# mims-harvard/GNNDelete

Hardware: AMD Instinct MI355X
Metric: Del-op train iters/sec (higher is better)
Workload: dtype f32; 1 GPU; synth-collab GCN 2-layer, 5.0% IN edge deletion, full-graph Del step (both_layerwise, mse_mean); num_nodes=235868, in_dim=128, hidden_dim=128, out_dim=64, train_edges_undirected=2122296, df_edges=53057, sdf_edges=1602188, spmm_nnz=1838056, S1=178921, S2=188697, hip_graph=True, matrix_products=fp32 matrix instruction (v_mfma_f32_32x32x2_f32), parallelism=single, ranks_seen=1

## Files before the change

gnndelete_amd/_lib.py:

```python
import ctypes
import os
import re

_HERE = os.path.dirname(os.path.abspath(__file__))
LIB_PATH = os.environ.get('GNNDELETE_HIP_LIB') or os.path.join(_HERE, 'lib', 'libgnndelete_hip.so')
HEADER_PATH = os.path.join(os.path.dirname(_HERE), 'include', 'gnndelete_hip.h')

_i32, _i64, _f32, _f64, _p = ctypes.c_int32, ctypes.c_int64, ctypes.c_float, ctypes.c_double, ctypes.c_void_p

ABI_VERSION = 9

PROTOTYPES = {
    'gd_abi_version': (ctypes.c_int, []),
    'gd_last_error_string': (ctypes.c_char_p, []),
    'gd_build_source_hash': (ctypes.c_char_p, []),
    'gd_matrix_split': (ctypes.c_int, []),
    'gd_set_matrix_split': (ctypes.c_int, [ctypes.c_int]),
    'gd_csr_from_coo_workspace': (_i64, [_i32, _i64]),
    'gd_csr_from_coo': (ctypes.c_int, [_p, _p, _i64, _i32, _p, _p, _p, _p, _p, _i64, _p]),
    'gd_gcn_norm_f32': (ctypes.c_int, [_p, _p, _i32, _p, _p]),
    'gd_spmm_csr_f32': (ctypes.c_int, [_p, _p, _p, _p, _i64, _p, _i64, _p, _f32, _i32, _i32, _p]),
    'gd_spmm_csr_balanced_f32': (ctypes.c_int, [_p, _i32, _p, _i32, _p, _p, _p, _i64, _p, _i64, _p, _f32, _p, _p, _i32,
                                                _i32, _i32, _p, _p]),
    'gd_spmm_csr_onepass_f32': (ctypes.c_int, [_p, _i32, _p, _p, _p, _i64, _p, _i64, _p, _f32, _p, _i32, _i32, _i32, _p, _p]),
# ... 47 lines not shown
    'gd_rowpair_mse_f32': (ctypes.c_int, [_p, _i64, _p, _i64, _i32, _p, _p, _i32, _p, _p, _p, _p, _i64, _i32,
                                          _p, _p, _p]),
    'gd_rowtarget_mse_workspace': (_i64, [_i32]),
    'gd_rowtarget_mse_f32': (ctypes.c_int, [_p, _i64, _p, _i32, _p, _p, _p, _p, _i32, _p, _i64, _p, _p, _p]),
    'gd_rowtarget_mse_pair_covers': (ctypes.c_int32, [_i32, _i32]),
    'gd_rowtarget_mse_pair_f32': (ctypes.c_int, [_p, _i64, _p, _i32, _p, _p, _p, _p, _i32, _p, _i64, _p, _p, _i64, _p, _i32, _p, _p, _p, _p, _i32, _p, _i64, _p, _p]),
    'gd_gemm_f32_workspace': (_i64, [_i32, _i32, _i32]),
    'gd_gemm_f32': (ctypes.c_int, [_p, _i64, _p, _i32, _p, _i32, _i32, _p, _p, _i64, _p, _p]),
    'gd_edge_dot_f32': (ctypes.c_int, [_p, _i64, _i32, _p, _p, _p, _i64, _p, _i64, _p, _p]),
    'gd_edge_dot_bwd_f32': (ctypes.c_int, [_p, _i64, _i32, _p, _p, _p, _i64, _p, _p, _i64, _p, _i64, _p]),
    'gd_rows_gemm_wgrad_adam_f32': (ctypes.c_int, [_p, _i64, _p, _p, _i64, _p, _p, _p, _i32, _i32, _i32, _p, _i32, _p,
                                                   _p, _p, _p, _p, _f64, _f64, _f64, _f64, _p]),
    'gd_rows_gemm_wgrad_blocks': (_i32, [_i32]),
    'gd_rows_gemm_wgrad_loss_f32': (ctypes.c_int, [_p, _i64, _p, _p, _i64, _p, _p, _p, _p, _p, _p, _i32, _i32, _i32, _p, _i32,
                                                   _p, _p, _p, _p, _p, _p, _f64, _f64, _f64, _f64, _p]),
    'gd_del_loss_bwd_blocks': (_i32, [_i32]),
    'gd_del_loss_bwd_f32': (ctypes.c_int, [_p, _i64, _p, _i32, _p, _i32, _p, _p, _p, _p, _p, _i64, _p, _i64, _p, _p]),
    'gd_del_loss_bwd_wgrad_f32': (ctypes.c_int, [_p, _i64, _p, _i32, _p, _i32, _p, _p, _p, _p, _p, _i64, _p, _i64, _p, _p, _p]),
    'gd_del_loss_bwd_wgrad_parts': (ctypes.c_int32, [_i32, _i32]),
    'gd_del_loss_bwd_wgrad_parts_f32': (ctypes.c_int, [_p, _i64, _p, _i32, _p, _i32, _p, _p, _p, _p, _p, _i64, _p, _i64, _p, _p, _i32, _p]),
    'gd_del1_loss_wgrad_covers': (ctypes.c_int32, [_i32, _i32]),
    'gd_del1_loss_wgrad_parts': (ctypes.c_int32, [_i32]),
    'gd_del1_chain_loss_wgrad_f32': (ctypes.c_int, [_p, _i64, _p, _i32, _p, _i32, _p, _i64, _p, _p, _p, _p, _p, _p, _i64, _i32, _p, _p, _p, _p, _p, _p, _p, _i32, _p]),
    'gd_del1_loss_wgrad_f32': (ctypes.c_int, [_p, _i64, _p, _i32, _p, _i32, _p, _i64, _p, _p, _p, _p, _p, _p, _i64, _p, _p, _i32, _p]),
    'gd_rowtarget_mse_blocks': (_i32, [_i32]),
    'gd_loss_finalize_f32': (ctypes.c_int, [_p, _i32, _p, _i32, _p, _p, _i32, _p, _p, _p]),
    'gd_pairs_sigmoid_mse_workspace': (_i64, [_i32, _i32]),
    'gd_pairs_sigmoid_mse_f32': (ctypes.c_int, [_p, _i64, _p, _i32, _i32, _p, _i64, _f32, _p, _p, _p, _p]),
    'gd_edgeprob_dec_workspace': (_i64, [_i64, _i32]),
    'gd_edgeprob_dec_f32': (ctypes.c_int, [_p, _i64, _i64, _i32, _p, _i64, _p, _i64, _i64, _f32, _p, _p, _p, _p, _p, _p, _p]),
    'gd_edge_incidence_workspace': (_i64, [_i64, _i64]),
    'gd_edge_incidence': (ctypes.c_int, [_p, _p, _i64, _i64, _p, _p, _p, _p, _i64, _p]),
    'gd_rows_add_f32': (ctypes.c_int, [_p, _i64, _i64, _p, _i32, _p, _i64, _f32, _i32, _p]),
    'gd_edgeprob_record_f32': (ctypes.c_int, [_p, _p, _f32, _f32, _p, _i32, _p, _p]),
    'gd_adam_at_f32': (ctypes.c_int, [_p, _p, _p, _p, _p, _i64, _f64, _f64, _f64, _f64, _p]),
    'gd_adam_f32': (ctypes.c_int, [_p, _p, _p, _p, _p, _i64, _f64, _f64, _f64, _f64, _p]),
    'gd_segment_softmax_f32': (ctypes.c_int, [_p, _p, _i32, _p, _p]),
    'gd_segment_softmax_bwd_f32': (ctypes.c_int, [_p, _p, _p, _i32, _p, _p]),
    'gd_rowpair_dot_f32': (ctypes.c_int, [_p, _i64, _p, _p, _i64, _p, _i64, _i32, _p, _p]),
    'gd_spmm_csr_onepass_aux_f32': (ctypes.c_int, [_p, _i32, _p, _p, _p, _p, _i64, _p, _i64, _p, _i32, _i32, _i32, _p, _p]),
    'gd_typed_wgrad_f32': (ctypes.c_int, [_p, _i32, _p, _p, _p, _p, _i64, _p, _i64, _i32, _i32, _i32, _p, _p]),
    'gd_typed_edge_dot_f32': (ctypes.c_int, [_p, _p, _p, _i64, _p, _i64, _p, _i64, _p, _i32, _i32, _i32, _p, _p]),
    'gd_comm_unique_id': (ctypes.c_int, [_p]),
    'gd_comm_init': (ctypes.c_int, [_p, _i32, _i32, ctypes.POINTER(ctypes.c_void_p)]),
    'gd_comm_destroy': (ctypes.c_int, [_p]),
    'gd_allreduce_f32': (ctypes.c_int, [_p, _i64, _p, _p]),
# ... 62 lines not shown
```

gnndelete_amd/csrc/common.h:

```cpp
#pragma once
#include <hip/hip_runtime.h>
#include <stdarg.h>
#include <stdint.h>
#include <stdio.h>

#include "gnndelete_hip.h"

namespace gd {

constexpr int kWave = 64;

char* error_buffer();
int matrix_split();
int ws_cu_count();
int rows_gemm_ws_try(const float* in, int64_t ld_in, const int32_t* idx, int32_t n_sel, const float* w, int32_t d_in, int32_t d_out,
                     int32_t trans_w, const float* bias, int32_t relu_in, const uint32_t* gate_bits, uint32_t* sign_out, float* out,
                     int64_t ld_out, float* save_in, void* stream, const float* in_alt, const uint8_t* sel, const float* u1,
                     const float* u2, float* o1, float* o2);

inline int fail(int code, const char* fmt, ...) {
  va_list ap;
  va_start(ap, fmt);
  vsnprintf(error_buffer(), 256, fmt, ap);
  va_end(ap);
// ... 32 lines not shown
  return __uint_as_float(r[0]) + __uint_as_float(r[1]);
}
__device__ __forceinline__ float xor16_sum(float v) {
  const auto r = __builtin_amdgcn_permlane16_swap(__float_as_uint(v), __float_as_uint(v), false, false);
  return __uint_as_float(r[0]) + __uint_as_float(r[1]);
}
template <int CTRL>
__device__ __forceinline__ float dpp_add(float v) {
  return v + __int_as_float(__builtin_amdgcn_update_dpp(0, __float_as_int(v), CTRL, 0xF, 0xF, true));
}
template <int LPR>
__device__ __forceinline__ float lanes_sum(float v) {
  if (LPR >= 2) v = dpp_add<0xB1>(v);
  if (LPR >= 4) v = dpp_add<0x4E>(v);
  if (LPR >= 8) v = dpp_add<0x141>(v);
  if (LPR >= 16) v = dpp_add<0x140>(v);
  if (LPR >= 32) v = xor16_sum(v);
  if (LPR >= 64) v = xor32_sum(v);
  return v;
}

template <int LPR>
__device__ __forceinline__ float4 f4_group_sum(float4 a) {
#pragma unroll
  for (int off = LPR; off < 8; off <<= 1) a = f4_add(a, f4_shfl_xor(a, off));
  if (LPR <= 8) a = make_float4(dpp_add<0x128>(a.x), dpp_add<0x128>(a.y), dpp_add<0x128>(a.z), dpp_add<0x128>(a.w));
  if (LPR <= 16) a = make_float4(xor16_sum(a.x), xor16_sum(a.y), xor16_sum(a.z), xor16_sum(a.w));
  if (LPR <= 32) a = make_float4(xor32_sum(a.x), xor32_sum(a.y), xor32_sum(a.z), xor32_sum(a.w));
  return a;
}
__device__ __forceinline__ float wave_sum(float v) {
#pragma unroll
  for (int off = 32; off > 0; off >>= 1) v += __shfl_xor(v, off);
  return v;
}

struct AdamScalars { float w1, b2, c2, neg_step, rs, eps; };
__device__ __forceinline__ AdamScalars adam_scalars(double lr, double beta1, double beta2, double eps, int t) {
  const double bc1 = 1.0 - pow(beta1, (double)t), bc2 = 1.0 - pow(beta2, (double)t);
  AdamScalars s;
  s.w1 = (float)(1.0 - beta1);
  s.b2 = (float)beta2;
  s.c2 = (float)(1.0 - beta2);
  s.neg_step = (float)(-(lr / bc1));
  s.rs = (float)sqrt(bc2);
  s.eps = (float)eps;
  return s;
}
__device__ __forceinline__ void adam_update(float& p, float& m, float& v, float g, const AdamScalars& s) {
#pragma clang fp contract(off)
  m = __builtin_fmaf(g - m, s.w1, m);
// ... 20 lines not shown
```

gnndelete_amd/csrc/del_fused.hip:

```cpp
#include <stdlib.h>

#include "common.h"

namespace gd {

using f32x16 = __attribute__((ext_vector_type(16))) float;

struct DelLoss {
  const int32_t* slot;
  const float* tm;
  const float* coef;
  const float* cnt_signed;
  float* partials;
};

template <int NT, bool WG>
__global__ __launch_bounds__(256, (NT == 2 && WG) ? 1 : 2) void del_loss_bwd_kernel(const float* __restrict__ p, int64_t ld_p,
                                                              const int32_t* __restrict__ idx, int32_t n_sel,
                                                              const float* __restrict__ w, DelLoss loss,
                                                              float* __restrict__ dz, int64_t ld_dz,
                                                              float* __restrict__ dp, int64_t ld_dp,
                                                              float* __restrict__ wg_partials) {
  constexpr int D = 32 * NT;
  constexpr int PB = D + 4;
// ... 532 lines not shown
  __syncthreads();
  for (int slot = blockIdx.x; slot < n_part; slot += gridDim.x) {
    float* const out = wg_partials + (int64_t)slot * D * D;
    const bool mine = slot == (int)blockIdx.x;
    for (int e = tid; e < D * D; e += 256) {
      const int i = e >> 7, c = e & 127, hf = c >> 6, ch = c & 63;
      out[e] = mine ? red[hf * D * H + i * H + ch] + red[(2 + hf) * D * H + i * H + ch] : 0.f;
    }
  }
  ls0 = wave_sum(ls0);
  ls1 = wave_sum(ls1);
  if (lane == 0) { lred[0][wave] = ls0; lred[1][wave] = ls1; }
  __syncthreads();
  if (tid == 0) {
    for (int slot = blockIdx.x; slot < n_part; slot += gridDim.x) {
      const bool mine = slot == (int)blockIdx.x;
      loss.partials[2 * slot + 0] = mine ? (lred[0][0] + lred[0][1]) + (lred[0][2] + lred[0][3]) : 0.f;
      loss.partials[2 * slot + 1] = mine ? (lred[1][0] + lred[1][1]) + (lred[1][2] + lred[1][3]) : 0.f;
    }
  }
}

struct ChainRank1 { const float* ra; const float* ua; const float* rb; const float* ub; };
template <bool RANK1>
__global__ __launch_bounds__(256) __attribute__((amdgpu_waves_per_eu(1, 1))) void del1_chain_ws_kernel(
    const float* __restrict__ p, int64_t ld_p, const int32_t* __restrict__ idx, int32_t n_sel, const float* __restrict__ w,
    float* __restrict__ z, int64_t ld_z, uint32_t* __restrict__ sign_io, DelLoss loss, const float* __restrict__ dt, int64_t ld_dt,
    const float* __restrict__ w_next, float* __restrict__ wg_partials, int32_t n_part, ChainRank1 r1) {
  constexpr int D = 128, H = 64, PTP = 144, PTZ = 80;
  constexpr int kTiles = 4 * (16 * PTP + 16 * PTZ);
  extern __shared__ __attribute__((aligned(16))) float wl[];
  __shared__ float lred[2][4];
  const int tid = threadIdx.x, lane = tid & 63;
  const int wave = __builtin_amdgcn_readfirstlane(tid >> 6);
  const int half = wave & 1, pair = wave >> 1, cb = H * half;
  const int r = lane & 15, kq = lane >> 4;
  float* const tp = wl + wave * (16 * PTP + 16 * PTZ);
  float* const tz = tp + 16 * PTP;
  float4* const wimg = reinterpret_cast<float4*>(wl + kTiles);
  float4* const w2img = wimg + 2 * 4 * 8 * 64;
  {
    float4 fv[16];
#pragma unroll
    for (int it = 0; it < 16; ++it) {
      const int e = tid + 256 * it;
      const int ln = e & 63, i_ = (e >> 6) & 7, t_ = (e >> 9) & 3, h_ = e >> 11;
      const float* src = w + (int64_t)(16 * i_ + 4 * (ln >> 4)) * D + 64 * h_ + 16 * t_ + (ln & 15);
// ... 33 lines not shown
  if (RANK1) {
#pragma unroll
    for (int t = 0; t < 4; ++t) {
      ua4[t] = *reinterpret_cast<const float4*>(r1.ua + cb + 16 * t + 4 * kq);
      ub4[t] = *reinterpret_cast<const float4*>(r1.ub + cb + 16 * t + 4 * kq);
    }
  }
  uint2 old_bits;
  float cf_raw, cn_raw;
  int32_t ls_cur;
  auto fetch_targets = [&](int32_t u) {
    const int uc = max(u, 0);
    const float* trow = loss.tm + (int64_t)uc * D + cb + 4 * kq;
#pragma unroll
    for (int t = 0; t < 4; ++t) tv[t] = *reinterpret_cast<const float4*>(trow + 16 * t);
    cf_raw = loss.coef[uc];
    cn_raw = loss.cnt_signed[uc];
    ls_cur = u;
  };
  auto fetch_rows = [&](int32_t row, int u) {
    const float4* src = reinterpret_cast<const float4*>(p + (int64_t)row * ld_p + 4 * kq);
#pragma unroll
    for (int i = 0; i < 8; ++i) x[i] = src[4 * i];
    const float4* dsrc = reinterpret_cast<const float4*>(dt + (int64_t)row * ld_dt + 4 * kq);
#pragma unroll
    for (int i = 0; i < 4; ++i) dv[i] = dsrc[4 * i];
    old_bits = *reinterpret_cast<const uint2*>(sign_io + (int64_t)slot_of(u) * 4 + 2 * half);
    if (RANK1) { ra_row = r1.ra[row]; rb_row = r1.rb[row]; }
  };
  if (u_lo < u_hi) {
    fetch_rows(row_n, u_lo);
    fetch_targets(ls_n);
    for (int u = u_lo; u < u_hi; ++u) {
      const int32_t row = row_n;
      const int s_a = min(u, n_units - 1) * 16 + r;
      const bool live = s_a < n_sel;
      const float livef = live ? 1.f : 0.f;
      row_n = row_nn;
      ls_n = ls_nn;
      row_nn = idx[slot_of(u + 2)];
      ls_nn = loss.slot[slot_of(u + 2)];
      f32x4w acc[4], dacc[4];
      {
        float4 wq[2][4];
#pragma unroll
        for (int t = 0; t < 4; ++t) wq[0][t] = wmine[(t * 8) * 64];
#pragma unroll
        for (int i = 0; i < 8; ++i) {
          if (i + 1 < 8) {
#pragma unroll
// ... 256 lines not shown
  GD_REQUIRE(aligned16(p) && aligned16(z) && aligned16(tm) && aligned16(w) && (!g_add || aligned16(g_add)) && aligned16(wgrad_partials),
             GD_E_ALIGN, "%s: unaligned", name);
  GD_REQUIRE(p != z && g_add != z, GD_E_DIM, "%s: z must not alias p or g_add (the two waves of a pair read whole rows)", name);
  hipStream_t s = (hipStream_t)stream;
  const DelLoss loss{loss_slot, tm, coef, cnt_signed, loss_partials};
  GD_REQUIRE(n_part >= 1 && n_part <= gd_rows_gemm_wgrad_blocks(n_sel), GD_E_DIM,
             "%s: n_part=%d outside [1, gd_rows_gemm_wgrad_blocks(n_sel)=%d]", name, n_part, gd_rows_gemm_wgrad_blocks(n_sel));
  const int grid = ws_cu_count() < n_part ? ws_cu_count() : n_part;
  constexpr int kLds = 4 * 128 * 64 * 4;
  if (g_add) {
    static const hipError_t a1 = hipFuncSetAttribute(reinterpret_cast<const void*>(&del1_loss_wgrad_ws_kernel<true>), hipFuncAttributeMaxDynamicSharedMemorySize, kLds);
    if (a1 != hipSuccess) return fail(-(int)a1, "%s: %s", name, hipGetErrorString(a1));
    hipLaunchKernelGGL((del1_loss_wgrad_ws_kernel<true>), dim3(grid), dim3(256), kLds, s, p, ld_p, idx, n_sel, w, z, ld_z, sign_out, loss, g_add,
                       ld_gadd, wgrad_partials, n_part);
  } else {
    static const hipError_t a0 = hipFuncSetAttribute(reinterpret_cast<const void*>(&del1_loss_wgrad_ws_kernel<false>), hipFuncAttributeMaxDynamicSharedMemorySize, kLds);
    if (a0 != hipSuccess) return fail(-(int)a0, "%s: %s", name, hipGetErrorString(a0));
    hipLaunchKernelGGL((del1_loss_wgrad_ws_kernel<false>), dim3(grid), dim3(256), kLds, s, p, ld_p, idx, n_sel, w, z, ld_z, sign_out, loss, nullptr,
                       0, wgrad_partials, n_part);
  }
  return launched("del1_loss_wgrad_ws");
}

extern "C" int gd_del1_chain_loss_wgrad_f32(const float* p, int64_t ld_p, const int32_t* idx, int32_t n_sel, const float* w, int32_t d,
                                            float* z, int64_t ld_z, uint32_t* sign_io, const int32_t* loss_slot, const float* tm,
                                            const float* coef, const float* cnt_signed, const float* dt, int64_t ld_dt, int32_t d_next,
                                            const float* w_next, const float* row_a, const float* col_a, const float* row_b,
                                            const float* col_b, float* loss_partials, float* wgrad_partials, int32_t n_part,
                                            void* stream) {
  using namespace gd;
  const char* name = "gd_del1_chain_loss_wgrad_f32";
  if (n_sel == 0) return GD_OK;
  GD_REQUIRE(p && idx && w && z && sign_io && loss_slot && tm && coef && cnt_signed && dt && w_next && loss_partials && wgrad_partials, GD_E_NULL,
             "%s: null pointer", name);
  GD_REQUIRE(d == 128 && d_next == 64, GD_E_DIM, "%s: widths %d / %d must be 128 / 64", name, d, d_next);
  GD_REQUIRE(ld_p >= d && ld_z >= d && ld_dt >= d_next && ld_p % 4 == 0 && ld_z % 4 == 0 && ld_dt % 4 == 0, GD_E_DIM, "%s: bad row strides", name);
  GD_REQUIRE(aligned16(p) && aligned16(z) && aligned16(tm) && aligned16(dt) && aligned16(wgrad_partials) && (reinterpret_cast<uintptr_t>(sign_io) & 7u) == 0,
             GD_E_ALIGN, "%s: unaligned", name);
  GD_REQUIRE(p != z && dt != z, GD_E_DIM, "%s: z must not alias p or dt", name);
  GD_REQUIRE(n_part >= 1 && n_part <= gd_rows_gemm_wgrad_blocks(n_sel), GD_E_DIM,
             "%s: n_part=%d outside [1, gd_rows_gemm_wgrad_blocks(n_sel)=%d]", name, n_part, gd_rows_gemm_wgrad_blocks(n_sel));
  const DelLoss loss{loss_slot, tm, coef, cnt_signed, loss_partials};
  const int grid = ws_cu_count() < n_part ? ws_cu_count() : n_part;
  constexpr int kLds = (4 * (16 * 144 + 16 * 80) + 128 * 128 + 64 * 128) * 4;
  const bool rank1 = row_a || col_a || row_b || col_b;
  GD_REQUIRE(!rank1 || (row_a && col_a && row_b && col_b && aligned16(col_a) && aligned16(col_b)), GD_E_NULL,
             "%s: the rank-1 terms come as four pointers (row_a, col_a, row_b, col_b; 16-byte aligned column vectors)", name);
  const ChainRank1 r1{row_a, col_a, row_b, col_b};
  if (rank1) {
    static const hipError_t at = hipFuncSetAttribute(reinterpret_cast<const void*>(&del1_chain_ws_kernel<true>), hipFuncAttributeMaxDynamicSharedMemorySize, kLds);
    if (at != hipSuccess) return fail(-(int)at, "%s: %s", name, hipGetErrorString(at));
    hipLaunchKernelGGL(del1_chain_ws_kernel<true>, dim3(grid), dim3(256), kLds, (hipStream_t)stream, p, ld_p, idx, n_sel, w, z, ld_z, sign_io, loss, dt,
                       ld_dt, w_next, wgrad_partials, n_part, r1);
  } else {
    static const hipError_t at = hipFuncSetAttribute(reinterpret_cast<const void*>(&del1_chain_ws_kernel<false>), hipFuncAttributeMaxDynamicSharedMemorySize, kLds);
    if (at != hipSuccess) return fail(-(int)at, "%s: %s", name, hipGetErrorString(at));
    hipLaunchKernelGGL(del1_chain_ws_kernel<false>, dim3(grid), dim3(256), kLds, (hipStream_t)stream, p, ld_p, idx, n_sel, w, z, ld_z, sign_io, loss, dt,
                       ld_dt, w_next, wgrad_partials, n_part, r1);
  }
  return launched("del1_chain_ws");
}
```

gnndelete_amd/engine.py:

```python
import os

import torch

from . import _lib, ops
from ._lib import check, ptr, stream_ptr
from .graph import graph_for
from .nn import GATConv, GCNConv, GINConv, RGCNConv, SAGEConv

LOSS_TYPES = ('both_all', 'both_layerwise', 'only2_layerwise', 'only2_all', 'only1')


def _loss_coefficients(loss_type, alpha):
    if loss_type in ('both_all', 'both_layerwise', 'only2_layerwise'):
        return alpha, 1.0 - alpha
    return alpha, 1.0


class _LayerTerms:

    def __init__(self, pos_edge, neg_edge, ni_mask, z_ori, coef_r, coef_l, reduction, row_range=None, d_norm=None):
        device = z_ori.device
        d = z_ori.shape[1]
        dn = d if d_norm is None else int(d_norm)
        pos, neg = pos_edge.to(device).long(), neg_edge.to(device).long()
# ... 316 lines not shown
        self._tail = (t1.folded and self.t2.folded and self.s1 > 0 and self.s2 > 0
                      and loss_type in ('both_layerwise', 'both_all') and not self._overlap and self.h % 2 == 0 and self.o % 2 == 0
                      and os.environ.get('GD_NO_STEP_TAIL') != '1'
                      and ((self._fuse_loss1 and self._fuse_l2)
                           or (self.h in (32, 64, 128) and self.o in (32, 64, 128) and os.environ.get('GD_TAIL_FUSED_ONLY') != '1')))
        self._tail_acc = [0, 0]
        self._arrive = torch.zeros(2, dtype=torch.int32, device=dev)
        self._fuse_wg2 = self._tail and self._fuse_l2 and os.environ.get('GD_NO_FUSED_WGRAD2') != '1'
        if self._fuse_wg2:
            self._lp2 = torch.zeros(2 * max(1, _lib.lib().gd_rows_gemm_wgrad_blocks(self.s2) + self.t2.outside_blocks()), **f32)
            self._lp2_blocks = _lib.lib().gd_del_loss_bwd_wgrad_parts(self.s2, self.o)
        self._fuse_del1 = bool(self._tail and self._fuse_loss1 and self._split1 and loss_type in ('both_layerwise', 'only1')
                               and _lib.lib().gd_del1_loss_wgrad_covers(self.s1, self.h))
        if self._fuse_del1:
            self._lp1_blocks = _lib.lib().gd_del1_loss_wgrad_parts(self.s1)
        self._chain1 = bool(self._fuse_del1 and loss_type == 'both_layerwise' and isinstance(conv2, (GCNConv, GINConv))
                            and self.h == 128 and self.o == 64 and os.environ.get('GD_DEL1_CHAIN') != '0')
        self._gat_bufs = None
        if (self._fuse_del1 and loss_type == 'both_layerwise' and isinstance(conv2, GATConv) and self.h == 128 and self.o == 64
                and self._mfma_weight(conv2.lin_src.weight) and os.environ.get('GD_NO_GAT_RANK1_EPILOGUE') != '1'
                and os.environ.get('GD_DEL1_CHAIN') != '0'):
            self._chain1 = True
            self._gat_bufs = {'dh': torch.zeros(n, self.o, **f32), 'da_src': torch.zeros(n, **f32), 'da_dst': torch.zeros(n, **f32)}
        self._dt2_keep = torch.zeros(n, self.o, **f32) if (self._chain1 and self._gat_bufs is None) else None
        self._side_w1 = bool(self._tail and self._fuse_loss1 and not self._fuse_del1 and loss_type == 'both_layerwise'
                             and self.s1 > 0 and not self._overlap and os.environ.get('GD_SMALL_SIDE_W1') == '1')
        if self._side_w1 and self._side is None:
            self._side = torch.cuda.Stream(device=dev)
        self._out_pair = bool(self._out1 and self._out2 and self._fuse_loss1 and self._fuse_l2 and loss_type != 'only2_all'
                              and _lib.lib().gd_rowtarget_mse_pair_covers(self.h, self.o) and os.environ.get('GD_NO_LOSS_PAIR') != '1')
        self._mode = {GCNConv: 'gcn', GINConv: 'gin', GATConv: 'gat', SAGEConv: 'sage', RGCNConv: 'rgcn'}[type(conv2)]
        self._gat_dots = os.environ.get('GD_NO_GAT_DOTS') != '1'
        self._gat_r1 = None
        if self._mode == 'gat':
            w2_ = conv2.lin_src.weight.detach()
            self._gat_r1 = ((conv2.att_src.detach().reshape(1, -1) @ w2_).reshape(-1).float().contiguous(),
                            (conv2.att_dst.detach().reshape(1, -1) @ w2_).reshape(-1).float().contiguous())
        if self._mode == 'rgcn':
            from .graph import TypedNodeCSR
            self.typed = TypedNodeCSR(edge_index, edge_type.to(dev), n, conv2.num_relations)
            self.typed_s1 = None
            if getattr(self, '_rgcn_rows_only', False) and self.s1 > 0:
                in1 = torch.zeros(n, dtype=torch.bool, device=dev)
                in1[self.idx1.long()] = True
                self.typed_s1 = self.typed.restrict_bwd(in1)
            self.graph = None
            self._hbuf = torch.zeros(n, self.h, **f32)
            self._dxbuf = torch.zeros(n, self.h, **f32)
            for c_, din, dout, tr in ((conv1, self.x.shape[1], self.h, 0), (conv2, self.h, self.o, 0), (conv2, self.o, self.h, 1)):
                if int(_lib.lib().gd_rgcn_tile_kl(din, dout, c_.num_blocks or 1, tr)) > 0 and os.environ.get('GD_RGCN_NODE_MAJOR') != '1':
                    tg_ = self.typed_s1 if (tr and self.typed_s1 is not None) else self.typed
                    if ops.rgcn_wave_form(din, dout, c_.num_blocks or 1, n, din) and self.typed.num_relations < 65536:
                        tg_.wave_plan(bool(tr))
                    else:
                        tg_.tile_plan(bool(tr))
                    ops.rgcn_packed_weight(c_.weight.detach(), c_.num_blocks or 1, din, dout, tr)
        else:
            gmode = {'gcn': 'gcn', 'gin': 'sum', 'gat': 'gat', 'sage': 'mean'}[self._mode]
            self.graph = graph_for(edge_index, n, gmode)
        if self._mode == 'sage':
            self._w2cat = torch.cat([conv2.lin_l.weight.detach(), conv2.lin_r.weight.detach()], 0).contiguous()
        self._rows_only = False
        gin_ok = self._mode == 'gin' and conv1.nn.out_features <= conv1.nn.in_features and conv2.nn.out_features <= conv2.nn.in_features
        if (affected_rows_only and (self._mode in ('gcn', 'gat', 'sage') or gin_ok) and self._split2 and self.s2 > 0
                and not self._out1 and not self._out2):
            g = self.graph
            in2 = torch.zeros(n, dtype=torch.bool, device=dev)
            in2[self.idx2.long()] = True
            in1_rows = torch.zeros(n, dtype=torch.bool, device=dev)
            in1_rows[self.idx1.long()] = True
            deg = (g.rowptr[1:] - g.rowptr[:-1]).long()
            erow = torch.repeat_interleave(torch.arange(n, device=dev), deg)
            closed = bool(in2[g.col.long()[in2[erow]]].all()) and bool(in2[self.idx1.long()].all())
            deg_t = (g.rowptr_t[1:] - g.rowptr_t[:-1]).long()
            erow_t = torch.repeat_interleave(torch.arange(n, device=dev), deg_t)
            closed = closed and bool(in2[g.col_t.long()[in1_rows[erow_t]]].all())
            if closed:
                from .graph import SplitPlan
                self._plan2 = SplitPlan(g.rowptr, rows=self.idx2)
                self._plan_t1 = SplitPlan(g.rowptr_t, rows=self.idx1)
                self._t1buf = torch.zeros(n, self.h, **f32)
                self._t1rbuf = torch.zeros(n, self.h, **f32) if self._mode == 'sage' else None
                self._t2buf = torch.zeros(n, self.o * (2 if self._mode == 'sage' else 1), **f32)
                self._dt2buf = torch.zeros(n, self.o, **f32)
                self._adots = torch.zeros(2, n, **f32)
                if self._split1:
                    self.pre1.zero_()
                self.p2.zero_()
                self._rows_only = True
        if self._rows_only and self._chain1 and self._dt2_keep is not None:
            self._dt2buf = self._dt2_keep
        self.cache_layer1 = cache_layer1
        if cache_layer1:
            with torch.no_grad():
                self._conv1_forward()
                if self._split1:
                    self.p1 = self.pre1
                else:
                    self.p1 = self.z1.clone()
                    if self.s1:
                        self.xs1.copy_(self.p1[self.idx1.long()])

    @staticmethod
# ... 139 lines not shown
                self._a_src, self._a_dst = ops.row_dots(h2, c.att_src, c.att_dst)
            self._h2 = h2
            _, self._rowmax, self._rowsum = ops.gat_forward_raw(self.graph, h2, self._a_src, self._a_dst, c.bias,
                                                                c.negative_slope, out=self.p2,
                                                                plan=self._plan2 if self._rows_only else None)

    def _conv2_backward_to_s1(self):
        c = self.model.conv2
        g = self.graph
        if self._mode == 'rgcn':
            if self.typed_s1 is not None:
                ops.rows_gemm(self.dz2, self.idx1, c.root.detach(), trans_w=True, out=self._dxbuf)
                ops.rgcn_typed_accumulate(self.typed_s1, self.dz2, c.weight.detach(), c.num_blocks or 1, 1, self._dxbuf)
            else:
                self._rgcn_conv(c, self.dz2, self._dxbuf, 1)
            ops.gate_rows(self._dxbuf, self.idx1, self.z1_pos, self.dh)
            return
        if self._mode == 'sage':
            self._spmm(True, g.val_t, self.dz2, self.dcat[:, :self.o], None, 0.0,
                       plan=self._plan_t1 if self._rows_only else None)
            dt2, w2 = self.dcat, self._w2cat
        elif self._mode in ('gcn', 'gin'):
            chain = self._chain1
            dt2 = self._dt2_keep if chain else torch.empty(self.n, self.o, dtype=torch.float32, device=self.x.device)
            if self._mode == 'gcn' and self._rows_only:
                dt2 = self._dt2buf
                self._spmm(True, g.val_t, self.dz2, dt2, None, 0.0, plan=self._plan_t1)
                w2 = c.lin.weight
            elif self._mode == 'gcn':
                self._spmm(True, g.val_t, self.dz2, dt2, None, 0.0)
                w2 = c.lin.weight
            elif self._rows_only:
                dt2 = self._dt2buf
                self._spmm(True, None, self.dz2, dt2, None, 1.0 + c.eps, plan=self._plan_t1)
                w2 = c.nn.weight
            else:
                self._spmm(True, None, self.dz2, dt2, None, 1.0 + c.eps)
                w2 = c.nn.weight
            if chain:
                return
        else:
            chain = self._chain1
            dt2, da_s, da_d = ops.gat_backward_raw(g, self._h2, self._a_src, self._a_dst, self._rowmax, self._rowsum,
                                                   self.dz2, c.negative_slope,
                                                   plan=self._plan2 if self._rows_only else None,
                                                   plan_t=self._plan_t1 if self._rows_only else None,
# ... 163 lines not shown
                    ptr(a2.m), ptr(a2.v), a1.lr, a1.betas[0], a1.betas[1], a1.eps, ptr(p1), n1, ptr(p2), n2, ptr(self.hist),
                    self.hist.shape[0], ptr(self.hist_pos), ptr(self.iter_ctr), ptr(self._arrive), stream_ptr(self.x.device)),
                    'gd_step_tail_parts_f32')
            elif self._overlap:
                with self._fork():
                    finalize()
                torch.cuda.current_stream().wait_stream(self._side)
            else:
                finalize()
            if self._user_wd2 is not None:
                self._user_wd2.data.copy_(self.wd2.data[:self._o_true, :self._o_true])

    def _del1_fused(self, g_add):
        self.adam1.applied += 1
        self._tail_acc[0] = 0
        if self._chain1:
            c2 = self.model.conv2
            if self._mode == 'gat':
                w_next, dt = c2.lin_src.weight.detach(), self._gat_bufs['dh']
                rank1 = (ptr(self._gat_bufs['da_src']), ptr(self._gat_r1[0]), ptr(self._gat_bufs['da_dst']), ptr(self._gat_r1[1]))
            else:
                w_next, dt = (c2.lin if self._mode == 'gcn' else c2.nn).weight.detach(), self._dt2_keep
                rank1 = (None, None, None, None)
            check(_lib.lib().gd_del1_chain_loss_wgrad_f32(
                ptr(self.pre1), self.pre1.stride(0), ptr(self.idx1), self.s1, ptr(self.wd1), self.h, ptr(self.z1), self.z1.stride(0),
                ptr(self.z1_pos), ptr(self._slot1), ptr(self.t1.tm), ptr(self.t1.coef), ptr(self._cnt_signed1), ptr(dt),
                dt.stride(0), self.o, ptr(w_next), *rank1, ptr(self._lp1), ptr(self.ws1), self._lp1_blocks,
                stream_ptr(self.x.device)), 'gd_del1_chain_loss_wgrad_f32')
            return
        check(_lib.lib().gd_del1_loss_wgrad_f32(
            ptr(self.pre1), self.pre1.stride(0), ptr(self.idx1), self.s1, ptr(self.wd1), self.h, ptr(self.z1), self.z1.stride(0),
            ptr(self.z1_pos), ptr(self._slot1), ptr(self.t1.tm), ptr(self.t1.coef), ptr(self._cnt_signed1), ptr(g_add),
            g_add.stride(0) if g_add is not None else 0, ptr(self._lp1), ptr(self.ws1), self._lp1_blocks, stream_ptr(self.x.device)),
            'gd_del1_loss_wgrad_f32')

    def _del2_fused(self):
        if self._fuse_wg2:
            check(_lib.lib().gd_del_loss_bwd_wgrad_parts_f32(
                ptr(self.p2), self.p2.stride(0), ptr(self.idx2), self.s2, ptr(self.wd2), self.o, ptr(self._slot2),
                ptr(self.t2.tm), ptr(self.t2.coef), ptr(self._cnt_signed2), None, self.o,
                ptr(self.dz2), self.dz2.stride(0), ptr(self._lp2), ptr(self.ws2), self._lp2_blocks, stream_ptr(self.x.device)),
                'gd_del_loss_bwd_wgrad_parts_f32')
            return
        check(_lib.lib().gd_del_loss_bwd_f32(
            ptr(self.p2), self.p2.stride(0), ptr(self.idx2), self.s2, ptr(self.wd2), self.o, ptr(self._slot2),
            ptr(self.t2.tm), ptr(self.t2.coef), ptr(self._cnt_signed2), ptr(self.dz2c), self.dz2c.stride(0),
# ... 113 lines not shown
```

gnndelete_amd/graph.py:

```python
import os

import torch

from . import _lib


CHUNK = 64


class SplitPlan:

    def __init__(self, rowptr, chunk=CHUNK, row_range=None, rows=None):
        dev = rowptr.device
        rpl = rowptr.long()
        if rows is not None:
            ids = rows.long()
        else:
            lo, hi = (0, rowptr.numel() - 1) if row_range is None else row_range
            ids = torch.arange(lo, hi, device=dev)
        r_start, r_end = rpl[ids], rpl[ids + 1]
        n = ids.numel()
        deg = r_end - r_start
        pieces = torch.clamp((deg + chunk - 1) // chunk, min=1)
        first = torch.cumsum(pieces, 0) - pieces
# ... 163 lines not shown
    def scratch(self, d, device):
        if self.n_slots == 0:
            return None
        buf = self._scratch.get(d)
        if buf is None:
            buf = torch.empty(self.n_slots, d, dtype=torch.float32, device=device)
            self._scratch[d] = buf
        return buf


class CSRGraph:

    def __init__(self, n, rowptr, col, val, rowptr_t, col_t, val_t, perm_t, mode):
        self.n, self.mode = n, mode
        self.rowptr, self.col, self.val = rowptr, col, val
        self.rowptr_t, self.col_t, self.val_t, self.perm_t = rowptr_t, col_t, val_t, perm_t
        self.nnz = int(col.shape[0])
        self.plan = SplitPlan(rowptr)
        self.plan_t = SplitPlan(rowptr_t)

    @property
    def device(self):
        return self.col.device


def csr_from_coo(src, dst, n):
    src, dst = src.long().contiguous(), dst.long().contiguous()
    dev, e = src.device, int(src.numel())
    L = _lib.lib()
    nbytes = int(L.gd_csr_from_coo_workspace(n, e))
    if nbytes < 0:
        raise ValueError('graph too large for int32 CSR indices')
    rowptr = torch.empty(n + 1, dtype=torch.int32, device=dev)
    col = torch.empty(e, dtype=torch.int32, device=dev)
    order = torch.empty(e, dtype=torch.int32, device=dev)
    status = torch.empty(1, dtype=torch.int32, device=dev)
    ws = torch.empty(nbytes, dtype=torch.uint8, device=dev)
    _lib.check(L.gd_csr_from_coo(_lib.ptr(src), _lib.ptr(dst), e, n, _lib.ptr(rowptr), _lib.ptr(col), _lib.ptr(order),
                                 _lib.ptr(status), _lib.ptr(ws), nbytes, _lib.stream_ptr(dev)), 'gd_csr_from_coo')
    if int(status):
        raise IndexError(f'edge_index has endpoints outside [0, {n})')
    return rowptr, col, order


def _sorted_csr(src, dst, n):
    if src.is_cuda:
# ... 351 lines not shown
```

include/gnndelete_hip.h:

```cpp
#ifndef GNNDELETE_HIP_H
#define GNNDELETE_HIP_H

#include <stdint.h>

#ifdef __cplusplus
extern "C" {
#endif

#define GD_ABI_VERSION 9

enum {
  GD_OK = 0,
  GD_E_NULL = 1,
  GD_E_DIM = 2,
  GD_E_ALIGN = 3,
  GD_E_WORKSPACE = 4
};

int gd_abi_version(void);
const char* gd_last_error_string(void);
const char* gd_build_source_hash(void);

#define GD_MATRIX_SPLIT_DEFAULT 0
int gd_matrix_split(void);
// ... 178 lines not shown
                        float* dz, int64_t ld_dz, float* dp, int64_t ld_dp, float* loss_partials, void* stream);

int gd_del_loss_bwd_wgrad_f32(const float* p, int64_t ld_p, const int32_t* idx, int32_t n_sel, const float* w, int32_t d,
                              const int32_t* loss_slot, const float* tm, const float* coef, const float* cnt_signed,
                              float* dz, int64_t ld_dz, float* dp, int64_t ld_dp, float* loss_partials,
                              float* wgrad_partials, void* stream);
int32_t gd_del_loss_bwd_wgrad_parts(int32_t n_sel, int32_t d);
int gd_del_loss_bwd_wgrad_parts_f32(const float* p, int64_t ld_p, const int32_t* idx, int32_t n_sel, const float* w, int32_t d,
                                    const int32_t* loss_slot, const float* tm, const float* coef, const float* cnt_signed,
                                    float* dz, int64_t ld_dz, float* dp, int64_t ld_dp, float* loss_partials,
                                    float* wgrad_partials, int32_t n_part, void* stream);

int32_t gd_del1_loss_wgrad_covers(int32_t n_sel, int32_t d);
int32_t gd_del1_loss_wgrad_parts(int32_t n_sel);
int gd_del1_loss_wgrad_f32(const float* p, int64_t ld_p, const int32_t* idx, int32_t n_sel, const float* w, int32_t d, float* z,
                           int64_t ld_z, uint32_t* sign_out, const int32_t* loss_slot, const float* tm, const float* coef,
                           const float* cnt_signed, const float* g_add, int64_t ld_gadd, float* loss_partials,
                           float* wgrad_partials, int32_t n_part, void* stream);
int gd_del1_chain_loss_wgrad_f32(const float* p, int64_t ld_p, const int32_t* idx, int32_t n_sel, const float* w, int32_t d, float* z,
                                 int64_t ld_z, uint32_t* sign_io, const int32_t* loss_slot, const float* tm, const float* coef,
                                 const float* cnt_signed, const float* dt, int64_t ld_dt, int32_t d_next, const float* w_next,
                                 const float* row_a, const float* col_a, const float* row_b, const float* col_b,
                                 float* loss_partials, float* wgrad_partials, int32_t n_part, void* stream);


int64_t gd_rowpair_mse_workspace(int32_t n_seg);
int gd_rowpair_mse_f32(const float* z, int64_t ld_z, const float* o, int64_t ld_o, int32_t d,
                       const int32_t* seg_ptr, const int32_t* seg_row, int32_t n_seg,
                       const int32_t* term_o, const float* term_w, const int32_t* term_kind,
                       float* dz, int64_t ld_dz, int32_t dz_compact,
                       float* sums, float* partials, void* stream);

int64_t gd_rowtarget_mse_workspace(int32_t n_rows);
int gd_rowtarget_mse_f32(const float* z, int64_t ld_z, const float* tm, int32_t d,
                         const int32_t* row_idx, const float* coef, const float* cnt, const int32_t* kind,
                         int32_t n_rows, float* dz, int64_t ld_dz, float* sums, float* partials, void* stream);
int32_t gd_rowtarget_mse_pair_covers(int32_t d_a, int32_t d_b);
int gd_rowtarget_mse_pair_f32(const float* z_a, int64_t ld_z_a, const float* tm_a, int32_t d_a, const int32_t* row_idx_a,
                              const float* coef_a, const float* cnt_a, const int32_t* kind_a, int32_t n_rows_a, float* dz_a,
                              int64_t ld_dz_a, float* partials_a, const float* z_b, int64_t ld_z_b, const float* tm_b, int32_t d_b,
                              const int32_t* row_idx_b, const float* coef_b, const float* cnt_b, const int32_t* kind_b,
                              int32_t n_rows_b, float* dz_b, int64_t ld_dz_b, float* partials_b, void* stream);

int32_t gd_rowtarget_mse_blocks(int32_t n_rows);
int gd_loss_finalize_f32(const float* partials1, int32_t n1, const float* partials2, int32_t n2,
                         const float* extra_sums, float* hist, int32_t capacity, int32_t* pos, int32_t* iter,
// ... 89 lines not shown
```

Before: 1821 iters/s.

## Store layer-2 transposed gradient in compact slot-indexed rows for GCN chain

For GCN with the fused layer-1 chain, the transposed SpMM producing dt2 now runs over a precomputed compact CSR holding only the selected layer-1 rows. It writes into an s1-row buffer indexed by slot instead of an n-row buffer indexed by node id. A new kernel variant reads dt by slot, replacing the split plan over the full transposed graph and shrinking the buffer. The group-sum reduction order in f4_group_sum is also reversed, applying the wide permlane swaps first and the narrow shuffles last.

```diff
diff --git a/gnndelete_amd/_lib.py b/gnndelete_amd/_lib.py
--- a/gnndelete_amd/_lib.py
+++ b/gnndelete_amd/_lib.py
@@ -93,6 +93,7 @@
     'gd_del1_loss_wgrad_covers': (ctypes.c_int32, [_i32, _i32]),
     'gd_del1_loss_wgrad_parts': (ctypes.c_int32, [_i32]),
     'gd_del1_chain_loss_wgrad_f32': (ctypes.c_int, [_p, _i64, _p, _i32, _p, _i32, _p, _i64, _p, _p, _p, _p, _p, _p, _i64, _i32, _p, _p, _p, _p, _p, _p, _p, _i32, _p]),
+    'gd_del1_chain_slot_loss_wgrad_f32': (ctypes.c_int, [_p, _i64, _p, _i32, _p, _i32, _p, _i64, _p, _p, _p, _p, _p, _p, _i64, _i32, _p, _p, _p, _i32, _p]),
     'gd_del1_loss_wgrad_f32': (ctypes.c_int, [_p, _i64, _p, _i32, _p, _i32, _p, _i64, _p, _p, _p, _p, _p, _p, _i64, _p, _p, _i32, _p]),
     'gd_rowtarget_mse_blocks': (_i32, [_i32]),
     'gd_loss_finalize_f32': (ctypes.c_int, [_p, _i32, _p, _i32, _p, _p, _i32, _p, _p, _p]),
diff --git a/gnndelete_amd/csrc/common.h b/gnndelete_amd/csrc/common.h
--- a/gnndelete_amd/csrc/common.h
+++ b/gnndelete_amd/csrc/common.h
@@ -78,11 +78,11 @@
 
 template <int LPR>
 __device__ __forceinline__ float4 f4_group_sum(float4 a) {
+  if (LPR <= 32) a = make_float4(xor32_sum(a.x), xor32_sum(a.y), xor32_sum(a.z), xor32_sum(a.w));
+  if (LPR <= 16) a = make_float4(xor16_sum(a.x), xor16_sum(a.y), xor16_sum(a.z), xor16_sum(a.w));
+  if (LPR <= 8) a = make_float4(dpp_add<0x128>(a.x), dpp_add<0x128>(a.y), dpp_add<0x128>(a.z), dpp_add<0x128>(a.w));
 #pragma unroll
-  for (int off = LPR; off < 8; off <<= 1) a = f4_add(a, f4_shfl_xor(a, off));
-  if (LPR <= 8) a = make_float4(dpp_add<0x128>(a.x), dpp_add<0x128>(a.y), dpp_add<0x128>(a.z), dpp_add<0x128>(a.w));
-  if (LPR <= 16) a = make_float4(xor16_sum(a.x), xor16_sum(a.y), xor16_sum(a.z), xor16_sum(a.w));
-  if (LPR <= 32) a = make_float4(xor32_sum(a.x), xor32_sum(a.y), xor32_sum(a.z), xor32_sum(a.w));
+  for (int off = 4; off >= LPR; off >>= 1) a = f4_add(a, f4_shfl_xor(a, off));
   return a;
 }
 __device__ __forceinline__ float wave_sum(float v) {
diff --git a/gnndelete_amd/csrc/del_fused.hip b/gnndelete_amd/csrc/del_fused.hip
--- a/gnndelete_amd/csrc/del_fused.hip
+++ b/gnndelete_amd/csrc/del_fused.hip
@@ -578,7 +578,7 @@
 }
 
 struct ChainRank1 { const float* ra; const float* ua; const float* rb; const float* ub; };
-template <bool RANK1>
+template <bool RANK1, bool DT_SLOT = false>
 __global__ __launch_bounds__(256) __attribute__((amdgpu_waves_per_eu(1, 1))) void del1_chain_ws_kernel(
     const float* __restrict__ p, int64_t ld_p, const int32_t* __restrict__ idx, int32_t n_sel, const float* __restrict__ w,
     float* __restrict__ z, int64_t ld_z, uint32_t* __restrict__ sign_io, DelLoss loss, const float* __restrict__ dt, int64_t ld_dt,
@@ -658,10 +658,11 @@
     const float4* src = reinterpret_cast<const float4*>(p + (int64_t)row * ld_p + 4 * kq);
 #pragma unroll
     for (int i = 0; i < 8; ++i) x[i] = src[4 * i];
-    const float4* dsrc = reinterpret_cast<const float4*>(dt + (int64_t)row * ld_dt + 4 * kq);
+    const int64_t slot = slot_of(u);
+    const float4* dsrc = reinterpret_cast<const float4*>(dt + (DT_SLOT ? slot : (int64_t)row) * ld_dt + 4 * kq);
 #pragma unroll
     for (int i = 0; i < 4; ++i) dv[i] = dsrc[4 * i];
-    old_bits = *reinterpret_cast<const uint2*>(sign_io + (int64_t)slot_of(u) * 4 + 2 * half);
+    old_bits = *reinterpret_cast<const uint2*>(sign_io + slot * 4 + 2 * half);
     if (RANK1) { ra_row = r1.ra[row]; rb_row = r1.rb[row]; }
   };
   if (u_lo < u_hi) {
@@ -964,14 +965,12 @@
   return launched("del1_loss_wgrad_ws");
 }
 
-extern "C" int gd_del1_chain_loss_wgrad_f32(const float* p, int64_t ld_p, const int32_t* idx, int32_t n_sel, const float* w, int32_t d,
-                                            float* z, int64_t ld_z, uint32_t* sign_io, const int32_t* loss_slot, const float* tm,
-                                            const float* coef, const float* cnt_signed, const float* dt, int64_t ld_dt, int32_t d_next,
-                                            const float* w_next, const float* row_a, const float* col_a, const float* row_b,
-                                            const float* col_b, float* loss_partials, float* wgrad_partials, int32_t n_part,
-                                            void* stream) {
-  using namespace gd;
-  const char* name = "gd_del1_chain_loss_wgrad_f32";
+namespace gd {
+static int launch_del1_chain(const char* name, bool dt_by_slot, const float* p, int64_t ld_p, const int32_t* idx, int32_t n_sel,
+                             const float* w, int32_t d, float* z, int64_t ld_z, uint32_t* sign_io, const int32_t* loss_slot,
+                             const float* tm, const float* coef, const float* cnt_signed, const float* dt, int64_t ld_dt,
+                             int32_t d_next, const float* w_next, const float* row_a, const float* col_a, const float* row_b,
+                             const float* col_b, float* loss_partials, float* wgrad_partials, int32_t n_part, void* stream) {
   if (n_sel == 0) return GD_OK;
   GD_REQUIRE(p && idx && w && z && sign_io && loss_slot && tm && coef && cnt_signed && dt && w_next && loss_partials && wgrad_partials, GD_E_NULL,
              "%s: null pointer", name);
@@ -989,7 +988,12 @@
   GD_REQUIRE(!rank1 || (row_a && col_a && row_b && col_b && aligned16(col_a) && aligned16(col_b)), GD_E_NULL,
              "%s: the rank-1 terms come as four pointers (row_a, col_a, row_b, col_b; 16-byte aligned column vectors)", name);
   const ChainRank1 r1{row_a, col_a, row_b, col_b};
-  if (rank1) {
+  if (dt_by_slot) {
+    static const hipError_t at = hipFuncSetAttribute(reinterpret_cast<const void*>(&del1_chain_ws_kernel<false, true>), hipFuncAttributeMaxDynamicSharedMemorySize, kLds);
+    if (at != hipSuccess) return fail(-(int)at, "%s: %s", name, hipGetErrorString(at));
+    hipLaunchKernelGGL((del1_chain_ws_kernel<false, true>), dim3(grid), dim3(256), kLds, (hipStream_t)stream, p, ld_p, idx, n_sel, w, z, ld_z, sign_io, loss,
+                       dt, ld_dt, w_next, wgrad_partials, n_part, r1);
+  } else if (rank1) {
     static const hipError_t at = hipFuncSetAttribute(reinterpret_cast<const void*>(&del1_chain_ws_kernel<true>), hipFuncAttributeMaxDynamicSharedMemorySize, kLds);
     if (at != hipSuccess) return fail(-(int)at, "%s: %s", name, hipGetErrorString(at));
     hipLaunchKernelGGL(del1_chain_ws_kernel<true>, dim3(grid), dim3(256), kLds, (hipStream_t)stream, p, ld_p, idx, n_sel, w, z, ld_z, sign_io, loss, dt,
@@ -1002,3 +1006,24 @@
   }
   return launched("del1_chain_ws");
 }
+}
+
+extern "C" int gd_del1_chain_loss_wgrad_f32(const float* p, int64_t ld_p, const int32_t* idx, int32_t n_sel, const float* w, int32_t d,
+                                            float* z, int64_t ld_z, uint32_t* sign_io, const int32_t* loss_slot, const float* tm,
+                                            const float* coef, const float* cnt_signed, const float* dt, int64_t ld_dt, int32_t d_next,
+                                            const float* w_next, const float* row_a, const float* col_a, const float* row_b,
+                                            const float* col_b, float* loss_partials, float* wgrad_partials, int32_t n_part,
+                                            void* stream) {
+  return gd::launch_del1_chain("gd_del1_chain_loss_wgrad_f32", false, p, ld_p, idx, n_sel, w, d, z, ld_z, sign_io, loss_slot, tm, coef, cnt_signed,
+                               dt, ld_dt, d_next, w_next, row_a, col_a, row_b, col_b, loss_partials, wgrad_partials, n_part, stream);
+}
+
+extern "C" int gd_del1_chain_slot_loss_wgrad_f32(const float* p, int64_t ld_p, const int32_t* idx, int32_t n_sel, const float* w, int32_t d,
+                                                 float* z, int64_t ld_z, uint32_t* sign_io, const int32_t* loss_slot, const float* tm,
+                                                 const float* coef, const float* cnt_signed, const float* dt_slots, int64_t ld_dt,
+                                                 int32_t d_next, const float* w_next, float* loss_partials, float* wgrad_partials,
+                                                 int32_t n_part, void* stream) {
+  return gd::launch_del1_chain("gd_del1_chain_slot_loss_wgrad_f32", true, p, ld_p, idx, n_sel, w, d, z, ld_z, sign_io, loss_slot, tm, coef,
+                               cnt_signed, dt_slots, ld_dt, d_next, w_next, nullptr, nullptr, nullptr, nullptr, loss_partials, wgrad_partials,
+                               n_part, stream);
+}
diff --git a/gnndelete_amd/engine.py b/gnndelete_amd/engine.py
--- a/gnndelete_amd/engine.py
+++ b/gnndelete_amd/engine.py
@@ -362,7 +362,9 @@
                 and os.environ.get('GD_DEL1_CHAIN') != '0'):
             self._chain1 = True
             self._gat_bufs = {'dh': torch.zeros(n, self.o, **f32), 'da_src': torch.zeros(n, **f32), 'da_dst': torch.zeros(n, **f32)}
-        self._dt2_keep = torch.zeros(n, self.o, **f32) if (self._chain1 and self._gat_bufs is None) else None
+        self._dt_slot = bool(self._chain1 and self._gat_bufs is None and isinstance(conv2, GCNConv))
+        self._dt2_keep = (torch.zeros(self.s1 if self._dt_slot else n, self.o, **f32)
+                          if (self._chain1 and self._gat_bufs is None) else None)
         self._side_w1 = bool(self._tail and self._fuse_loss1 and not self._fuse_del1 and loss_type == 'both_layerwise'
                              and self.s1 > 0 and not self._overlap and os.environ.get('GD_SMALL_SIDE_W1') == '1')
         if self._side_w1 and self._side is None:
@@ -398,6 +400,10 @@
         else:
             gmode = {'gcn': 'gcn', 'gin': 'sum', 'gat': 'gat', 'sage': 'mean'}[self._mode]
             self.graph = graph_for(edge_index, n, gmode)
+        self._csr_t1 = None
+        if self._dt_slot:
+            from .graph import CompactRowsCSR
+            self._csr_t1 = CompactRowsCSR(self.graph.rowptr_t, self.graph.col_t, self.graph.val_t, self.idx1)
         if self._mode == 'sage':
             self._w2cat = torch.cat([conv2.lin_l.weight.detach(), conv2.lin_r.weight.detach()], 0).contiguous()
         self._rows_only = False
@@ -418,7 +424,7 @@
             if closed:
                 from .graph import SplitPlan
                 self._plan2 = SplitPlan(g.rowptr, rows=self.idx2)
-                self._plan_t1 = SplitPlan(g.rowptr_t, rows=self.idx1)
+                self._plan_t1 = None if self._dt_slot else SplitPlan(g.rowptr_t, rows=self.idx1)
                 self._t1buf = torch.zeros(n, self.h, **f32)
                 self._t1rbuf = torch.zeros(n, self.h, **f32) if self._mode == 'sage' else None
                 self._t2buf = torch.zeros(n, self.o * (2 if self._mode == 'sage' else 1), **f32)
@@ -604,6 +610,10 @@
             dt2, w2 = self.dcat, self._w2cat
         elif self._mode in ('gcn', 'gin'):
             chain = self._chain1
+            if self._dt_slot:
+                t = self._csr_t1
+                ops._spmm_raw(t.rowptr, t.col, t.val, self.dz2, None, 0.0, t.n_rows, t.plan, out=self._dt2_keep)
+                return
             dt2 = self._dt2_keep if chain else torch.empty(self.n, self.o, dtype=torch.float32, device=self.x.device)
             if self._mode == 'gcn' and self._rows_only:
                 dt2 = self._dt2buf
@@ -813,6 +823,13 @@
             else:
                 w_next, dt = (c2.lin if self._mode == 'gcn' else c2.nn).weight.detach(), self._dt2_keep
                 rank1 = (None, None, None, None)
+            if self._dt_slot:
+                check(_lib.lib().gd_del1_chain_slot_loss_wgrad_f32(
+                    ptr(self.pre1), self.pre1.stride(0), ptr(self.idx1), self.s1, ptr(self.wd1), self.h, ptr(self.z1), self.z1.stride(0),
+                    ptr(self.z1_pos), ptr(self._slot1), ptr(self.t1.tm), ptr(self.t1.coef), ptr(self._cnt_signed1), ptr(dt),
+                    dt.stride(0), self.o, ptr(w_next), ptr(self._lp1), ptr(self.ws1), self._lp1_blocks,
+                    stream_ptr(self.x.device)), 'gd_del1_chain_slot_loss_wgrad_f32')
+                return
             check(_lib.lib().gd_del1_chain_loss_wgrad_f32(
                 ptr(self.pre1), self.pre1.stride(0), ptr(self.idx1), self.s1, ptr(self.wd1), self.h, ptr(self.z1), self.z1.stride(0),
                 ptr(self.z1_pos), ptr(self._slot1), ptr(self.t1.tm), ptr(self.t1.coef), ptr(self._cnt_signed1), ptr(dt),
diff --git a/gnndelete_amd/graph.py b/gnndelete_amd/graph.py
--- a/gnndelete_amd/graph.py
+++ b/gnndelete_amd/graph.py
@@ -209,6 +209,27 @@
     @property
     def device(self):
         return self.col.device
+
+
+class CompactRowsCSR:
+
+    def __init__(self, rowptr, col, val, rows):
+        dev = rowptr.device
+        ids = rows.long()
+        rpl = rowptr.long()
+        start = rpl[ids]
+        deg = rpl[ids + 1] - start
+        ptr = torch.zeros(ids.numel() + 1, dtype=torch.long, device=dev)
+        ptr[1:] = torch.cumsum(deg, 0)
+        nnz = int(ptr[-1])
+        if nnz >= 2 ** 31:
+            raise ValueError('graph too large for int32 CSR indices')
+        take = torch.repeat_interleave(start - ptr[:-1], deg) + torch.arange(nnz, device=dev)
+        self.n_rows = int(ids.numel())
+        self.rowptr = ptr.to(torch.int32)
+        self.col = col[take].contiguous()
+        self.val = val[take].contiguous() if val is not None else None
+        self.plan = SplitPlan(self.rowptr)
 
 
 def csr_from_coo(src, dst, n):
diff --git a/include/gnndelete_hip.h b/include/gnndelete_hip.h
--- a/include/gnndelete_hip.h
+++ b/include/gnndelete_hip.h
@@ -224,6 +224,10 @@
                                  const float* cnt_signed, const float* dt, int64_t ld_dt, int32_t d_next, const float* w_next,
                                  const float* row_a, const float* col_a, const float* row_b, const float* col_b,
                                  float* loss_partials, float* wgrad_partials, int32_t n_part, void* stream);
+int gd_del1_chain_slot_loss_wgrad_f32(const float* p, int64_t ld_p, const int32_t* idx, int32_t n_sel, const float* w, int32_t d, float* z,
+                                      int64_t ld_z, uint32_t* sign_io, const int32_t* loss_slot, const float* tm, const float* coef,
+                                      const float* cnt_signed, const float* dt_slots, int64_t ld_dt, int32_t d_next, const float* w_next,
+                                      float* loss_partials, float* wgrad_partials, int32_t n_part, void* stream);
 
 
 int64_t gd_rowpair_mse_workspace(int32_t n_seg);
```

Result: faster. 1859 iters/s (median of 6 runs) (+2.1%).
